# ducha-aiki/mods

Measured on AMD Instinct MI355X. Metric: image-pairs/sec (1024x768, HessAff+RootSIFT over the affine view ladder, MFMA FGINN match, LO-RANSAC H), higher is better.
Workload: dtype f32 (detect/describe) + u8 on the int8 matrix cores (distance matrix)

## Files before the change

mods_amd/csrc/engine.hip:

```cpp
#include <atomic>
#include <math.h>
#include <stdio.h>
#include <algorithm>
#include <chrono>
#include <map>
#include <unordered_set>
#include <mutex>
#include <dlfcn.h>
#include <string>
#include "engine_api.hpp"

#ifdef MODSX_DUP_BUILD
namespace mx {
int dup_count(int cls) {
  static const long mask = getenv("MODSX_DUP") ? strtol(getenv("MODSX_DUP"), nullptr, 0) : 0;
  return 1 + (int)((mask >> cls) & 1);
}
}
#endif
namespace mx {

static thread_local std::string g_err;
void set_error(const std::string &s) { g_err = s; }
static std::atomic<int> g_busyContexts{0};
// ... 362 lines not shown

static int cv_round(double v) { return (int)lrint(v); }

struct SigmaPlan {
  int levels;
  float sigmaStep;
  float curSigma[8];
  float incSigma[8];
};

static SigmaPlan make_sigma_plan(const modsx_hessaff_params &p) {
  SigmaPlan s;
  s.levels = p.numberOfScales + 2;
  s.sigmaStep = powf(2.0f, 1.0f / (float)p.numberOfScales);
  float cur = p.initialSigma;
  s.curSigma[0] = cur; s.incSigma[0] = 0;
  for (int i = 1; i < s.levels; i++) {
    s.incSigma[i] = cur * sqrtf(s.sigmaStep * s.sigmaStep - 1.0f);
    cur *= s.sigmaStep;
    s.curSigma[i] = cur;
  }
  return s;
}

static int fill_taps(BlurBatch &b, float sigma) {
  int n = blur_ksize(sigma);
  if (n > MAX_TAPS) { set_error("pyramid blur kernel larger than 17 taps is not supported"); return MODSX_ERR_ARG; }
  std::vector<float> k = gaussian_kernel(n, sigma);
  b.n = n;
  for (int i = 0; i < n; i++) b.k[i] = k[i];
  return MODSX_OK;
}

int build_pyramids(modsx_ctx *c, const modsx_image *const *imgs, int n, const modsx_hessaff_params &p,
                   bool singleOctaveFromFirstLevel) {
  if (n <= 0 || n > MAXB) { set_error("batch size"); return MODSX_ERR_ARG; }
  if (p.numberOfScales < 1 || p.numberOfScales > 6) { set_error("numberOfScales"); return MODSX_ERR_ARG; }
  if (p.detectorType != MODSX_DET_HESSIAN && p.detectorType != MODSX_DET_DOG && p.detectorType != MODSX_DET_HARRIS) {
    set_error("detectorType must be Hessian (0), DoG (1) or Harris (2)");
    return MODSX_ERR_ARG;
  }
  const bool hess = p.detectorType == MODSX_DET_HESSIAN;
  const SigmaPlan sp = make_sigma_plan(p);
  const int L = sp.levels;
  const int minSize = 2 * p.border + 2;
  int maxOct = 0;
  for (int i = 0; i < n; i++) {
    Pyramid &py = c->pyr[i];
    py.nOct = 0;
    int rows = imgs[i]->rows, cols = imgs[i]->cols;
    float pd = 1.0f;
    size_t total = 0;
    while (rows > minSize && cols > minSize && py.nOct < 24) {
      Octave &o = py.oct[py.nOct++];
      o.rows = rows; o.cols = cols; o.pixelDistance = pd;
      total += (size_t)2 * L * rows * cols;
      pd *= 2.0;
      rows = cv_round(rows * 0.5); cols = cv_round(cols * 0.5);
      if (singleOctaveFromFirstLevel) break;
    }
    if (!py.store.ensure(total * sizeof(float) + 64)) return MODSX_ERR_NOMEM;
    float *ptr = (float *)py.store.p;
    for (int o = 0; o < py.nOct; o++) {
      size_t npx = (size_t)py.oct[o].rows * py.oct[o].cols;
      for (int l = 0; l < L; l++) { py.oct[o].blur[l] = ptr; ptr += npx; }
      for (int l = 0; l < L; l++) { py.oct[o].resp[l] = ptr; ptr += npx; }
    }
    maxOct = std::max(maxOct, py.nOct);
  }
  hipStream_t s = c->stream;
  for (int o = 0; o < maxOct; o++) {
    BlurBatch bb;
    memset(&bb, 0, sizeof bb);
    int nj = 0, mr = 0, mc = 0;
    if (o == 0) {
      const float curSigma0 = 0.5f;
      const bool preBlur = !singleOctaveFromFirstLevel && p.initialSigma > curSigma0;
      if (preBlur) {
        float sigma = sqrtf(p.initialSigma * p.initialSigma - curSigma0 * curSigma0);
        int rc = fill_taps(bb, sigma);
        if (rc) return rc;
      }
      for (int i = 0; i < n; i++) {
        if (c->pyr[i].nOct <= 0) continue;
        Octave &oc = c->pyr[i].oct[0];
        BlurJob &j = bb.j[nj++];
        j.src = imgs[i]->d; j.blur = oc.blur[0]; j.resp = hess ? oc.resp[0] : nullptr; j.rows = oc.rows; j.cols = oc.cols;
        j.norm = sp.curSigma[0] * sp.curSigma[0];
        mr = std::max(mr, oc.rows); mc = std::max(mc, oc.cols);
        if (!preBlur) {
          MX_HIP(hipMemcpyAsync(oc.blur[0], imgs[i]->d, (size_t)oc.rows * oc.cols * 4, hipMemcpyDeviceToDevice, s));
          j.src = oc.blur[0];
        }
      }
      double px = 0;
      for (int q = 0; q < nj; q++) px += (double)bb.j[q].rows * bb.j[q].cols;
      if (nj) {
        if (preBlur) { ProfScope ps(c, K_BLUR_HESS, px * 12); launch_blur_hess(s, bb, nj, mr, mc); }
        else if (hess) { ProfScope ps(c, K_HESSIAN, px * 8); launch_hessian(s, bb, nj, mr, mc); }
      }
    } else {
      ResizeBatch rb;
      memset(&rb, 0, sizeof rb);
      for (int i = 0; i < n; i++) {
        if (c->pyr[i].nOct <= o) continue;
        Octave &pv = c->pyr[i].oct[o - 1], &oc = c->pyr[i].oct[o];
        ResizeJob &r = rb.j[nj];
        r.src = pv.blur[p.numberOfScales]; r.dst = oc.blur[0];
        r.srows = pv.rows; r.scols = pv.cols; r.drows = oc.rows; r.dcols = oc.cols;
        r.resp = hess ? oc.resp[0] : nullptr; r.norm = sp.curSigma[0] * sp.curSigma[0];
        BlurJob &j = bb.j[nj++];
        j.src = oc.blur[0]; j.blur = nullptr; j.resp = oc.resp[0]; j.rows = oc.rows; j.cols = oc.cols;
        j.norm = sp.curSigma[0] * sp.curSigma[0];
        mr = std::max(mr, oc.rows); mc = std::max(mc, oc.cols);
      }
      if (nj) {
        double spx = 0, dpx = 0;
        for (int q = 0; q < nj; q++) { spx += (double)rb.j[q].srows * rb.j[q].scols; dpx += (double)rb.j[q].drows * rb.j[q].dcols; }
        { ProfScope ps(c, K_RESIZE, (spx + dpx) * 4 + dpx * 4); launch_resize_half(s, rb, nj, mr, mc); }
      }
    }
    if (!nj) continue;
    for (int l = 1; l < L; l++) {
      BlurBatch b2;
      memset(&b2, 0, sizeof b2);
      int rc = fill_taps(b2, sp.incSigma[l]);
      if (rc) return rc;
      int k = 0;
      for (int i = 0; i < n; i++) {
        if (c->pyr[i].nOct <= o) continue;
        Octave &oc = c->pyr[i].oct[o];
        BlurJob &j = b2.j[k++];
        j.src = oc.blur[l - 1]; j.blur = oc.blur[l]; j.resp = hess ? oc.resp[l] : nullptr; j.rows = oc.rows; j.cols = oc.cols;
        j.norm = sp.curSigma[l] * sp.curSigma[l];
      }
      double px = 0;
      for (int q = 0; q < k; q++) px += (double)b2.j[q].rows * b2.j[q].cols;
      ProfScope ps(c, K_BLUR_HESS, px * 12);
      launch_blur_hess(s, b2, k, mr, mc);
    }
    if (!hess) {
      for (int l = 0; l < L; l++) {
        const float norm = sp.curSigma[l] * sp.curSigma[l];
        const float sigma = p.detectorType == MODSX_DET_DOG ? norm : sqrtf((float)(0.6 * norm));
        const int nt = blur_ksize(sigma);
        if (2 * nt > 2 * 4096) { set_error("response blur kernel too large"); return MODSX_ERR_ARG; }
        if (!c->viewTaps.ensure((size_t)L * 2 * 4100 * 4) || !c->hViewTaps.ensure((size_t)L * 2 * 4100 * 4)) return MODSX_ERR_NOMEM;
        float *dT = (float *)c->viewTaps.p + (size_t)l * 2 * 4100, *hT = (float *)c->hViewTaps.p + (size_t)l * 2 * 4100;
        bool tapsUp = false;
        for (int i = 0; i < n; i++) {
          if (c->pyr[i].nOct <= o) continue;
          Octave &oc = c->pyr[i].oct[o];
          const int rows = oc.rows, cols = oc.cols;
          const size_t npx = (size_t)rows * cols;
          if (!c->scratchA.ensure(npx * 4 * 8)) return MODSX_ERR_NOMEM;
          float *buf = (float *)c->scratchA.p, *tmp = buf, *a = buf + npx, *b = buf + 2 * npx, *cc = buf + 3 * npx;
          float *ba = buf + 4 * npx, *bb2 = buf + 5 * npx, *bc = buf + 6 * npx;
          const int nx = cols == 1 ? 1 : nt, ny = rows == 1 ? 1 : nt;
          if (!tapsUp || nx != nt || ny != nt) {
            std::vector<float> kx = gaussian_kernel(nx, sigma), ky = gaussian_kernel(ny, sigma);
            if (tapsUp) MX_HIP(ctx_sync(c));
            memcpy(hT, kx.data(), nx * 4); memcpy(hT + nx, ky.data(), ny * 4);
            MX_HIP(ctx_copy(c, dT, hT, (size_t)(nx + ny) * 4, hipMemcpyHostToDevice));
            tapsUp = nx == nt && ny == nt;
          }
          auto blur = [&](const float *src, float *dst) {
            if (nt == 1) { MX_HIP(hipMemcpyAsync(dst, src, npx * 4, hipMemcpyDeviceToDevice, s)); return MODSX_OK; }
            launch_blur_pass(s, src, tmp, rows, cols, dT, nx, 0, 1);
            launch_blur_pass(s, tmp, dst, rows, cols, dT + nx, ny, 1, 1);
            return MODSX_OK;
          };
          if (p.detectorType == MODSX_DET_DOG) {
            int rc = blur(oc.blur[l], a);
            if (rc) return rc;
            launch_sub(s, oc.blur[l], a, oc.resp[l], npx);
          } else {
            launch_grad_products(s, oc.blur[l], rows, cols, a, b, cc);
            int rc = blur(a, ba);
            if (!rc) rc = blur(b, bb2);
            if (!rc) rc = blur(cc, bc);
            if (rc) return rc;
            launch_harris_combine(s, ba, bb2, bc, (float)(0.6 * norm), oc.resp[l], npx);
          }
        }
      }
    }
  }
  MX_HIP(hipGetLastError());
  return MODSX_OK;
}

static const unsigned CAND_CAP = 1u << 21;

int detect_scalespace_batch(modsx_ctx *c, const modsx_image *const *imgs, int n, const modsx_hessaff_params &p,
                            std::vector<modsx_sskp> *out) {
  int rc = build_pyramids(c, imgs, n, p, false);
  if (rc) return rc;
  hipStream_t s = c->stream;
  if (!c->cand.ensure((size_t)CAND_CAP * sizeof(Candidate)) || !c->nmsQueue.ensure((size_t)CAND_CAP * 16)) return MODSX_ERR_NOMEM;
  if (!c->counter.ensure((NMS_QUEUES + 1) * 128)) return MODSX_ERR_NOMEM;
  MX_HIP(hipMemsetAsync(c->counter.p, 0, 128 + NMS_QUEUES * 128, s));
  bool queuesClean = true;
  NmsBatch nb;
  memset(&nb, 0, sizeof nb);
  nb.edgeScoreThreshold = (p.edgeEigenValueRatio + 1.0f) * (p.edgeEigenValueRatio + 1.0f) / p.edgeEigenValueRatio;
  float finalTh = p.threshold;
  float posTh = (float)(0.8 * finalTh);
  float negTh = -posTh;
  if (p.detectorType == MODSX_DET_HESSIAN) finalTh = p.threshold * p.threshold;
  if (p.mode != MODSX_FIXED_TH) finalTh = posTh = negTh = 0.0f;
  nb.posTh = posTh; nb.negTh = negTh; nb.finalTh = finalTh; nb.border = p.border; nb.detType = p.detectorType;
  int maxOct = 0;
  for (int i = 0; i < n; i++) maxOct = std::max(maxOct, c->pyr[i].nOct);
  const bool perOctave = p.numberOfScales == 3 && !getenv("MODSX_NMS_PER_LEVEL");
  std::vector<NmsJob> hjobs;
  std::vector<int> hpfx(1, 0), hfirst;
  double px = 0;
  auto flush = [&](bool last) -> int {
    const int nj = (int)hjobs.size();
    if (!nj) return MODSX_OK;
    const int np = (int)hpfx.size() - 1;
    const size_t jobBytes = (size_t)nj * sizeof(NmsJob), pfxBytes = (size_t)(np + 1) * 4, firstBytes = (size_t)std::max<size_t>(1, hfirst.size()) * 4;
    if (!c->nmsJobs.ensure(jobBytes + pfxBytes + firstBytes + 64)) return MODSX_ERR_NOMEM;
    if (!c->hNms.ensure(jobBytes + pfxBytes + firstBytes)) return MODSX_ERR_NOMEM;
    memcpy(c->hNms.p, hjobs.data(), jobBytes);
    memcpy((char *)c->hNms.p + jobBytes, hpfx.data(), pfxBytes);
    if (!hfirst.empty()) memcpy((char *)c->hNms.p + jobBytes + pfxBytes, hfirst.data(), hfirst.size() * 4);
    MX_HIP(ctx_copy(c, c->nmsJobs.p, c->hNms.p, jobBytes + pfxBytes + firstBytes, hipMemcpyHostToDevice));
    if (!c->tileJob.ensure((size_t)hpfx.back() * 4 + 4)) return MODSX_ERR_NOMEM;
    const int *dPfx = (const int *)((char *)c->nmsJobs.p + jobBytes);
    launch_expand_tiles(s, dPfx, np, (int *)c->tileJob.p);
    {
      ProfScope ps(c, K_NMS, px * 12);
      if (!queuesClean) MX_HIP(hipMemsetAsync((unsigned *)c->counter.p + 32, 0, NMS_QUEUES * 128, s));
      queuesClean = false;
      launch_nms(s, nb, (const NmsJob *)c->nmsJobs.p, dPfx, (const int *)c->tileJob.p, nj,
                 hpfx.back(), (int4 *)c->nmsQueue.p, (unsigned *)c->counter.p + 32, CAND_CAP, (Candidate *)c->cand.p,
                 (unsigned *)c->counter.p, CAND_CAP, perOctave ? (const int *)((char *)c->nmsJobs.p + jobBytes + pfxBytes) : nullptr,
                 p.numberOfScales);
    }
    if (!last) MX_HIP(ctx_sync(c));
    hjobs.clear(); hpfx.assign(1, 0); hfirst.clear(); px = 0;
    return MODSX_OK;
  };
  for (int o = 0; o < maxOct; o++)
    for (int i = 0; i < n; i++) {
      if (c->pyr[i].nOct <= o) continue;
      Octave &oc = c->pyr[i].oct[o];
      const int w = oc.cols - 2 * p.border, h = oc.rows - 2 * p.border;
      if (w <= 0 || h <= 0) continue;
      if ((int)hjobs.size() + p.numberOfScales > NMS_MAXJ) { int rcf = flush(false); if (rcf) return rcf; }
      const int tiles = ((w + 63) / 64) * ((h + NMS_TILE_ROWS - 1) / NMS_TILE_ROWS);
      if (perOctave) { hfirst.push_back((int)hjobs.size()); hpfx.push_back(hpfx.back() + tiles); }
      for (int l = 1; l <= p.numberOfScales; l++) {
        NmsJob j;
        j.low = oc.resp[l - 1]; j.cur = oc.resp[l]; j.high = oc.resp[l + 1]; j.blur = oc.blur[l];
        j.rows = oc.rows; j.cols = oc.cols; j.img = i; j.octave = o; j.level = l; j.pad = 0;
        hjobs.push_back(j);
        if (!perOctave) hpfx.push_back(hpfx.back() + tiles);
        px += (double)oc.rows * oc.cols;
      }
    }
  { int rcf = flush(true); if (rcf) return rcf; }
  static const bool deviceOrder = getenv("MODSX_DEVICE_ORDER") != nullptr && atoi(getenv("MODSX_DEVICE_ORDER")) != 0;
  if (deviceOrder) {
    typedef size_t (*temp_fn)(unsigned);
    typedef int (*order_fn)(hipStream_t, const Candidate *, const unsigned *, unsigned, unsigned long long *, unsigned long long *, unsigned *, unsigned *,
                            void *, size_t, unsigned long long *, unsigned *, unsigned, unsigned *, Candidate *, unsigned *);
    static temp_fn cand_sort_temp_bytes = nullptr;
    static order_fn launch_cand_order = nullptr;
    static std::once_flag candOnce;
    std::call_once(candOnce, [] {
      Dl_info di;
      std::string path = "libmodsx_cand.so";
      if (dladdr((const void *)&modsx_create, &di) && di.dli_fname) {
        const std::string self(di.dli_fname);
        const size_t sl = self.rfind('/');
        if (sl != std::string::npos) path = self.substr(0, sl + 1) + "libmodsx_cand.so";
// ... 1195 lines not shown
```

mods_amd/csrc/engine.hpp:

```cpp
#pragma once
#include <hip/hip_runtime.h>
#include <stdint.h>
#include <stdlib.h>
#include <string.h>
#include <string>
#include <vector>
#include "../../include/modsx.h"
#include "kmath.hpp"

namespace mx {

#ifndef MODSX_MAXB
#define MODSX_MAXB 32
#endif
constexpr int MAXB = MODSX_MAXB;
constexpr int PAIR_GROUP = 4;
constexpr int NMS_MAXJ = 1024;
constexpr int MAX_TAPS = 17;

struct BlurJob {
  const float *src;
  float *blur;
  float *resp;
  int rows, cols;
  float norm;
  int pad;
};
struct BlurBatch {
  int n;
  float k[MAX_TAPS];
  BlurJob j[MAXB];
  int nj;
  int tile0[MAXB + 1];
};
struct ResizeJob {
  const float *src;
  float *dst;
  float *resp;
  int srows, scols, drows, dcols;
  float norm;
  int pad;
};
struct ResizeBatch { ResizeJob j[MAXB]; int nj; int tile0[MAXB + 1]; };
struct NmsJob {
  const float *low, *cur, *high, *blur;
  int rows, cols, img, octave, level, pad;
};
struct NmsBatch {
  float posTh, negTh, finalTh;
  int border;
  double edgeScoreThreshold;
  int detType, pad;
};
struct Candidate {
  int img, octave, level, type;
  int r0, c0, r, c;
  float b0, b1, b2, val;
};

struct AffJob {
  const float *blur;
  int rows, cols;
  float x, y, s, pixelDistance;
};
struct AffOut { float u11, u12, u21, u22; int ok; int iters; };

struct OriJob {
// ... 51 lines not shown
};

struct MatchRow {
  int t0, t1, nless, nbad;
  int tj;
  float dj;
  float d0, d1;
};
static_assert(sizeof(MatchRow) == 32, "match rows are 32 bytes");

struct DevBuf {
  void *p = nullptr;
  size_t cap = 0;
  bool ensure(size_t bytes);
  void release();
};
struct PinBuf {
  void *p = nullptr;
  size_t cap = 0;
  bool ensure(size_t bytes);
  void release();
};

struct Octave {
  int rows, cols;
  float pixelDistance;
  float *blur[8];
  float *resp[8];
};
struct Pyramid {
  int nOct = 0;
  Octave oct[24];
  DevBuf store;
};

void set_error(const std::string &s);
bool gpu_shared();
struct CtxBusy { modsx_ctx *c; explicit CtxBusy(modsx_ctx *c); ~CtxBusy(); CtxBusy(const CtxBusy &) = delete; CtxBusy &operator=(const CtxBusy &) = delete; };
hipError_t ctx_copy(modsx_ctx *c, void *dst, const void *src, size_t bytes, hipMemcpyKind kind);
hipError_t ctx_sync(modsx_ctx *c);
unsigned ctx_mark(modsx_ctx *c);
bool ctx_mark_reached(modsx_ctx *c, unsigned seq);
hipError_t ctx_wait_mark(modsx_ctx *c, unsigned seq);
bool host_wait_runtime();
int host_cpus_per_rank();
#define MX_HIP(expr)                                                                          \
  do {                                                                                        \
    hipError_t e_ = (expr);                                                                   \
    if (e_ != hipSuccess) {                                                                   \
      mx::set_error(std::string(#expr) + ": " + hipGetErrorString(e_));                       \
      return MODSX_ERR_DEVICE;                                                                \
    }                                                                                         \
  } while (0)

std::vector<float> gaussian_kernel(int n, double sigma);
int blur_ksize(float sigma);
void gauss_mask(float *mask, int size);
void circular_gauss_mask(float *mask, int size, float sigma);
const double *atan_lut_host();
inline bool check_borders_host(int w, int h, float ofsx, float ofsy, float a11, float a12, float a21, float a22, int rw, int rh) {
  return check_borders(w, h, ofsx, ofsy, a11, a12, a21, a22, rw, rh);
}
bool invert3(const double *S, double *t);
void rectify(double &a11, double &a12, double &a21, double &a22);

void launch_blur_hess(hipStream_t s, const BlurBatch &b, int nj, int maxRows, int maxCols);
void launch_hessian(hipStream_t s, const BlurBatch &b, int nj, int maxRows, int maxCols);
void launch_resize_half(hipStream_t s, const ResizeBatch &b, int nj, int maxRows, int maxCols);
void launch_nms(hipStream_t s, const NmsBatch &b, const NmsJob *jobs, const int *tilePrefix, const int *tileJob, int nj,
                int nTiles, int4 *queue, unsigned *qcount, unsigned qcap, Candidate *out, unsigned *counter, unsigned cap,
                const int *octFirst = nullptr, int levelsPerOctave = 0);
size_t cand_sort_temp_bytes(unsigned nsort);
int launch_cand_order(hipStream_t s, const Candidate *cand, const unsigned *counter, unsigned nsort, unsigned long long *keys,
                      unsigned long long *keys2, unsigned *idx, unsigned *idx2, void *temp, size_t tempBytes, unsigned long long *tabKey,
                      unsigned *tabRank, unsigned tabSize, unsigned *slotOf, Candidate *out, unsigned *outCount);
constexpr int NMS_QUEUES = 64;
constexpr int NMS_TILE_ROWS = 16;
void launch_gray(hipStream_t s, const void *src, float *dst, size_t n, int channels, int dtype);
void launch_baumberg(hipStream_t s, const AffJob *jobs, AffOut *out, int n, const float *mask, int W, int maxIter,
                     float convTh, float affInitialSigma);
constexpr int ATAN_CASES = 2048 + 64;
constexpr int ORI_NV = 1344;
void launch_orientation(hipStream_t s, const OriJob *jobs, float *out, int n, const ImgRef *imgs,
                        const unsigned short *maskIdx, const float *maskW,
                        const unsigned char *binTab, int doHalf, double th, int maxAngles);
void launch_trunc_u8(hipStream_t s, const float *src, uint8_t *dst, size_t n);
size_t mser_sort_blocks(const int *rows, int n);
void launch_mser_sort(hipStream_t s, const uint8_t *const *u8, const int *rows, const int *cols, const size_t *ordOfs, int n, int *blockHist,
                      int *start, int *order);
void launch_expand_blur_tiles(hipStream_t s, const DescJob *jobs, const int *prefixRows, const int *prefixCols, int nJobs,
                              const int *needTab, BlurTile *tilesRows, BlurTile *tilesCols, float2 *rowStarts);
void launch_sample_rows(hipStream_t s, const DescJob *jobs, const BlurTile *tiles, int nTiles, const ImgRef *imgs, const float *taps,
                        const int *needTab, float *dst, const float2 *rowStarts, float *dstGrid);
void launch_blur_cols(hipStream_t s, const BlurTile *tiles, int nTiles, const float *taps, const int *needTab, const float *src,
                      float *dst);
void launch_expand_tiles(hipStream_t s, const int *prefix, int nJobs, int *tileJob);
void launch_patch_sample(hipStream_t s, const DescJob *jobs, const int *tilePrefix, const int *tileJob, int nTiles,
                         const ImgRef *imgs, float *scratch);
void launch_patch_blur(hipStream_t s, const DescJob *jobs, const int *tilePrefix, const int *tileJob, int nTiles,
                       const float *taps, const int *needTab, const float *src, float *dst, int pass);
void launch_describe(hipStream_t s, const DescJob *jobs, int n, const ImgRef *imgs, const float *grid,
                     const int *needTab, const float *coordTab,
                     const float *mask, const unsigned short *maskIdx, int nmask, const float *oTab, const int *bins,
                     const double *wts, int photoNorm, int descTypes, int nOut, double maxBin, const DescOut &outs);
// ... 121 lines not shown
```

mods_amd/csrc/engine_api.hpp:

```cpp
#pragma once
#include <functional>
#include <string>
#include <vector>
#include "engine.hpp"

struct modsx_comm;

namespace mx {
const char *last_error();
void prof_collect(modsx_ctx *c);
void prof_reset(modsx_ctx *c, bool enable);
modsx_ctx *ctx_create(int device_id);
void ctx_destroy(modsx_ctx *c);
int build_pyramids(modsx_ctx *c, const modsx_image *const *imgs, int n, const modsx_hessaff_params &p,
                   bool singleOctaveFromFirstLevel);
int detect_scalespace_batch(modsx_ctx *c, const modsx_image *const *imgs, int n, const modsx_hessaff_params &p,
                            std::vector<modsx_sskp> *out);
int detect_keypoints_batch(modsx_ctx *c, const modsx_image *const *imgs, int n, const modsx_hessaff_params &par,
                           const double *tilts, const double *zooms, std::vector<modsx_keypoint> *out);
void detect_affine_regions(const modsx_keypoint *kps, int n, int img_id, int det_type, modsx_region *out);
int detect_orientation_batch(modsx_ctx *c, const modsx_image *const *imgs, int n, const std::vector<modsx_region> *in,
                             double mrSize, int patchSize, int doHalfSIFT, int maxAngNum, double th, int addUpRight,
                             std::vector<modsx_region> *out);
int reproject_regions(modsx_region *regs, int n, const double *H, int orig_w, int orig_h);
int reproject_regions_box(modsx_region *regs, int n, const double *H, int orig_w, int orig_h, double boxk);
struct DescSet {
  int n = 1;
  int type[MODSX_MAX_DESC] = {MODSX_DESC_ROOT_SIFT, 0, 0, 0};
  double ratio[MODSX_MAX_DESC] = {0, 0, 0, 0};
  bool forceHalf = false;
  bool half() const { for (int i = 0; i < n; i++) if (type[i] >= 2) return true; return forceHalf; }
  int packed() const { int p = 0; for (int i = 0; i < n; i++) p |= (type[i] & 15) << (4 * i); return p; }
};
int resolve_descs(const modsx_pair_params &pp, const modsx_ladder_step *st, DescSet &ds);
void desc_class_order(const DescSet &ds, int *ord);
int describe_batch(modsx_ctx *c, const modsx_image *const *imgs, int n, const std::vector<modsx_region> *regs,
                   double mrSize, int patchSize, int fast, int photoNorm, int descType, double maxBin,
                   float *const *descHost, float *const *devF, uint8_t *const *devU8, const DescSet *ds = nullptr,
                   uint8_t *const *const *devU8x = nullptr);
struct ProfScopeFwd;
int set_vs_pars(const double *scale_set, int ns, const double *tilt_set, int nt, double phi_base, double InitSigma,
                int doBlur, modsx_view *par, int cap, modsx_view *prev, int *nprev, int cap_prev);
int synth_view(modsx_ctx *c, const modsx_image *gray, const modsx_view &v, modsx_image **out, double *H, int *identity,
               int slot = -1);
int detect_describe_items(modsx_ctx *c, const modsx_image *const *itemImg, const int *itemView, int nitems, const modsx_view *views,
                          const modsx_pair_params &pp, std::vector<modsx_region> &regs,
                          float *devF, uint8_t *devU8, size_t devCapRegions, float *hostDesc, int *itemCounts,
                          const DescSet *ds = nullptr, uint8_t *const *devU8x = nullptr);
// ... 115 lines not shown
```

mods_amd/csrc/kernels_pyramid.hip:

```cpp
#include "engine.hpp"

namespace mx {

constexpr int TW = 64;
constexpr int TMP_W = TW + 4;

MX_D int find_job(const int *tile0, int nj, int t) {
  int j = 0;
  while (j + 1 < nj && t >= tile0[j + 1]) j++;
  return j;
}

typedef float f2 __attribute__((ext_vector_type(2)));

template <int R, int TH>
__global__ __launch_bounds__(256) void k_blur_hess(BlurBatch batch) {
  constexpr int BLR_H = TH + 4;
  const int ji = find_job(batch.tile0, batch.nj, blockIdx.x);
  const BlurJob jb = batch.j[ji];
  const int rows = jb.rows, cols = jb.cols;
  const int lt = blockIdx.x - batch.tile0[ji], ntx = (cols + TW - 1) / TW;
  const int tx0 = (lt % ntx) * TW, ty0 = (lt / ntx) * TH;
  constexpr int n = 2 * R + 1;
  constexpr int sh = BLR_H + 2 * R, sw = TMP_W + 2 * R;
  static_assert(sh % 2 == 0, "the input tile is parked as row pairs");
  constexpr int SW = (sw + 3) & ~3;
  __shared__ __attribute__((aligned(16))) float src[sh * SW];
  __shared__ __attribute__((aligned(16))) float tmp[sh * TMP_W];
  float *blr = src;
  const int tid = threadIdx.x;
  {
    constexpr int PER = (sh * sw + 255) / 256;
    float t[PER];
#pragma unroll
    for (int u = 0; u < PER; u++) {
      const int i = tid + 256 * u, ii = i < sh * sw ? i : sh * sw - 1;
      const int ly = ii / sw, lx = ii - ly * sw;
      int gy = ty0 - 1 - R + ly, gx = tx0 - 1 - R + lx;
      gy = gy < 0 ? 0 : (gy > rows - 1 ? rows - 1 : gy);
      gx = gx < 0 ? 0 : (gx > cols - 1 ? cols - 1 : gx);
      t[u] = as_global(jb.src)[__umul24((unsigned)gy, (unsigned)cols) + (unsigned)gx];
    }
#pragma unroll
    for (int u = 0; u < PER; u++) {
      const int i = tid + 256 * u;
      if (i < sh * sw) { const int ly = i / sw, lx = i - ly * sw; src[(ly >> 1) * (2 * SW) + 2 * lx + (ly & 1)] = t[u]; }
    }
  }
  __syncthreads();
  for (int i = tid; i < (sh / 2) * (TMP_W / 4); i += 256) {
    const int lp = i / (TMP_W / 4), g = i - lp * (TMP_W / 4);
    const f2 *S = reinterpret_cast<const f2 *>(src) + lp * SW + 4 * g;
    f2 w[4 + 2 * R];
#pragma unroll
    for (int q = 0; q < (4 + 2 * R) / 2; q++) {
      const float4 t = *reinterpret_cast<const float4 *>(S + 2 * q);
      w[2 * q] = (f2){t.x, t.y}; w[2 * q + 1] = (f2){t.z, t.w};
    }
    f2 v[4];
#pragma unroll
    for (int o = 0; o < 4; o++) {
      if (n <= 5) {
        v[o] = w[o + R] * batch.k[R];
#pragma unroll
        for (int j = 1; j <= R; j++) v[o] = v[o] + (w[o + R - j] + w[o + R + j]) * batch.k[R + j];
      } else {
        v[o] = (f2){0.f, 0.f};
#pragma unroll
        for (int j = 0; j < n; j++) v[o] = v[o] + w[o + j] * batch.k[j];
      }
    }
    *reinterpret_cast<float4 *>(tmp + (2 * lp) * TMP_W + 4 * g) = make_float4(v[0].x, v[1].x, v[2].x, v[3].x);
    *reinterpret_cast<float4 *>(tmp + (2 * lp + 1) * TMP_W + 4 * g) = make_float4(v[0].y, v[1].y, v[2].y, v[3].y);
  }
  __syncthreads();
  for (int i = tid; i < (BLR_H / 4) * (TMP_W / 2); i += 256) {
    const int gy = i / (TMP_W / 2), lx = 2 * (i - gy * (TMP_W / 2));
    const float *S = tmp + (4 * gy) * TMP_W + lx;
    f2 w[4 + 2 * R];
#pragma unroll
    for (int q = 0; q < 4 + 2 * R; q++) w[q] = *reinterpret_cast<const f2 *>(S + q * TMP_W);
#pragma unroll
    for (int o = 0; o < 4; o++) {
      f2 v = w[o + R] * batch.k[R] + (f2){0.f, 0.f};
#pragma unroll
      for (int j = 1; j <= R; j++) v = v + (w[o + R + j] + w[o + R - j]) * batch.k[R + j];
      *reinterpret_cast<f2 *>(blr + (4 * gy + o) * TMP_W + lx) = v;
    }
  }
  __syncthreads();
  const float norm2 = jb.norm * jb.norm;
  for (int i = tid; i < TH * TW; i += 256) {
    const int ly = i / TW, lx = i - ly * TW;
    const int gy = ty0 + ly, gx = tx0 + lx;
    if (gy >= rows || gx >= cols) continue;
    const float *B = blr + (ly + 1) * TMP_W + (lx + 1);
    const unsigned gofs = __umul24((unsigned)gy, (unsigned)cols) + (unsigned)gx;
    jb.blur[gofs] = B[0];
    if (jb.resp) {
      float o = 0.f;
      if (gy >= 1 && gy < rows - 1 && gx >= 1 && gx < cols - 1) {
        const float v11 = B[-TMP_W - 1], v12 = B[-TMP_W], v13 = B[-TMP_W + 1];
        const float v21 = B[-1], v22 = B[0], v23 = B[1];
        const float v31 = B[TMP_W - 1], v32 = B[TMP_W], v33 = B[TMP_W + 1];
        float Lxx = (v21 - 2 * v22 + v23);
        float Lyy = (v12 - 2 * v22 + v32);
        float Lxy = (v13 - v11 + v31 - v33) / 4.0f;
        o = (Lxx * Lyy - Lxy * Lxy) * norm2;
      }
      jb.resp[gofs] = o;
    }
  }
}

__global__ __launch_bounds__(256) void k_hessian(BlurBatch batch) {
  const int ji = find_job(batch.tile0, batch.nj, blockIdx.x);
  const BlurJob jb = batch.j[ji];
  const int rows = jb.rows, cols = jb.cols;
  const int lt = blockIdx.x - batch.tile0[ji], ntx = (cols + 63) / 64;
  const int gx = (lt % ntx) * 64 + (threadIdx.x & 63), gy = (lt / ntx) * 4 + (threadIdx.x >> 6);
  if (gx >= cols || gy >= rows) return;
  float o = 0.f;
  if (gy >= 1 && gy < rows - 1 && gx >= 1 && gx < cols - 1) {
    const float *B = jb.src + (size_t)gy * cols + gx;
    const float v11 = B[-cols - 1], v12 = B[-cols], v13 = B[-cols + 1];
    const float v21 = B[-1], v22 = B[0], v23 = B[1];
    const float v31 = B[cols - 1], v32 = B[cols], v33 = B[cols + 1];
    float Lxx = (v21 - 2 * v22 + v23);
    float Lyy = (v12 - 2 * v22 + v32);
    float Lxy = (v13 - v11 + v31 - v33) / 4.0f;
    o = (Lxx * Lyy - Lxy * Lxy) * (jb.norm * jb.norm);
  }
  jb.resp[(size_t)gy * cols + gx] = o;
}

MX_D float resize_half_px(const float *src, int sr, int sc, int dx, int dy) {
  const int sy0 = dy * 2, sx0 = dx * 2;
  float out;
  if (sy0 >= sr) out = 0.f;
  else if (sy0 + 2 <= sr && dx < sc / 2) {
    const float *S = src + (size_t)sy0 * sc + sx0;
    float sum = 0.f;
    sum = sum + (((S[0] + S[1]) + S[sc]) + S[sc + 1]);
// ... 368 lines not shown
  unsigned n = qcount[32 * sq];
  n = n < qsub ? n : qsub;
  const int lane = threadIdx.x & 63;
  for (unsigned i0 = blockIdx.x * 256; i0 < n; i0 += gridDim.x * 256) {
    const unsigned i = i0 + threadIdx.x;
    Candidate k;
    bool ok = false;
    if (i < n) {
      const int4 q = queue[(size_t)sq * qsub + i];
      ok = nms_refine(batch, jobs[q.x], q.y, q.z, k);
    }
    const unsigned long long m = __ballot(ok);
    if (m) {
      unsigned base = 0;
      const int leader = __ffsll((long long)m) - 1;
      if (lane == leader) base = atomicAdd(counter, (unsigned)__popcll(m));
      base = __shfl(base, leader);
      const unsigned slot = base + (unsigned)__popcll(m & ((1ull << lane) - 1ull));
      if (ok && slot < cap) out[slot] = k;
    }
  }
}

void launch_nms(hipStream_t s, const NmsBatch &b, const NmsJob *jobs, const int *tilePrefix, const int *tileJob, int nj,
                int nTiles, int4 *queue, unsigned *qcount, unsigned qcap, Candidate *out, unsigned *counter, unsigned cap,
                const int *octFirst, int levelsPerOctave) {
  if (nj <= 0 || nTiles <= 0) return;
  if (octFirst && levelsPerOctave == 3)
    hipLaunchKernelGGL(k_nms_localize_oct<3>, dim3(nTiles), dim3(256), 0, s, b, jobs, octFirst, tilePrefix, tileJob, queue, qcount, qcap, counter + 1);
  else
  hipLaunchKernelGGL(k_nms_localize, dim3(nTiles), dim3(256), 0, s, b, jobs, tilePrefix, tileJob, queue, qcount, qcap, counter + 1);
  hipLaunchKernelGGL(k_nms_refine, dim3(NMS_REFINE_BLOCKS, NMS_QUEUES), dim3(256), 0, s, b, jobs, queue, qcount, qcap, out, counter, cap);
}
__global__ void k_trunc_u8(const float *src, uint8_t *dst, size_t n) {
  const size_t i = ((size_t)blockIdx.x * blockDim.x + threadIdx.x) * 4;
  if (i + 3 < n) {
    const float4 v = *reinterpret_cast<const float4 *>(src + i);
    const unsigned p = (unsigned)(uint8_t)v.x | ((unsigned)(uint8_t)v.y << 8) | ((unsigned)(uint8_t)v.z << 16) | ((unsigned)(uint8_t)v.w << 24);
    *reinterpret_cast<unsigned *>(dst + i) = p;
  } else {
    for (size_t k = i; k < n; k++) dst[k] = (uint8_t)src[k];
  }
}
void launch_trunc_u8(hipStream_t s, const float *src, uint8_t *dst, size_t n) {
  if (!n) return;
  const size_t threads = (n + 3) / 4;
  hipLaunchKernelGGL(k_trunc_u8, dim3((unsigned)((threads + 255) / 256)), dim3(256), 0, s, src, dst, n);
}
constexpr int MSB_ROWS = 8;
struct MserSortBatch {
  const uint8_t *u8[MAXB];
  int rows[MAXB], cols[MAXB], blk0[MAXB + 1];
  unsigned long long ordOfs[MAXB];
  int n;
};
MX_D int mser_view_of(const MserSortBatch &b, int blk) {
  int v = 0;
  while (v + 1 < b.n && blk >= b.blk0[v + 1]) v++;
  return v;
}
__global__ __launch_bounds__(64) void k_mser_hist(MserSortBatch b, int *blockHist) {
  __shared__ int h[256];
  const int blk = blockIdx.x, v = mser_view_of(b, blk), lane = threadIdx.x;
  for (int i = lane; i < 256; i += 64) h[i] = 0;
  __syncthreads();
  const int r0 = (blk - b.blk0[v]) * MSB_ROWS, r1 = min(r0 + MSB_ROWS, b.rows[v]), cols = b.cols[v];
// ... 74 lines not shown
```

Before: 217.7.

## Fuse NMS scan and next-octave seeding into the blur-Hessian pyramid kernel

The blur+Hessian kernel now does more of the detector's work itself. It runs the scale-space extremum scan on the previous level while the current response tile is still in shared memory, and pushes candidates straight into the NMS refine queues. It also writes the next octave's half-resolution base level and its Hessian response from the last blurred level, which removes the separate resize pass. The global tile load is restructured into per-wave row loads. This removes the separate localize kernel and the extra passes over response and blur memory, at the cost of a heavier, more register- and shared-memory-hungry kernel, more complex code, and an environment variable to fall back to the old path.

Result: slower. 208.8 (-4.1%).

```diff
diff --git a/mods_amd/csrc/engine.hip b/mods_amd/csrc/engine.hip
--- a/mods_amd/csrc/engine.hip
+++ b/mods_amd/csrc/engine.hip
@@ -418,19 +418,27 @@
   return MODSX_OK;
 }
 
-int build_pyramids(modsx_ctx *c, const modsx_image *const *imgs, int n, const modsx_hessaff_params &p,
-                   bool singleOctaveFromFirstLevel) {
+enum { PYR_SEP_SCAN = 1, PYR_SEP_SEED = 2 };
+static int pyramid_separate() {
+#ifdef MODSX_DUP_BUILD
+  return PYR_SEP_SCAN | PYR_SEP_SEED;
+#endif
+  const char *e = getenv("MODSX_PYRAMID_SEPARATE");
+  if (!e || !*e || !strcmp(e, "0")) return 0;
+  if (!strcmp(e, "scan")) return PYR_SEP_SCAN;
+  if (!strcmp(e, "seed")) return PYR_SEP_SEED;
+  return PYR_SEP_SCAN | PYR_SEP_SEED;
+}
+
+int plan_pyramids(modsx_ctx *c, const modsx_image *const *imgs, int n, const modsx_hessaff_params &p, bool singleOctaveFromFirstLevel) {
   if (n <= 0 || n > MAXB) { set_error("batch size"); return MODSX_ERR_ARG; }
   if (p.numberOfScales < 1 || p.numberOfScales > 6) { set_error("numberOfScales"); return MODSX_ERR_ARG; }
   if (p.detectorType != MODSX_DET_HESSIAN && p.detectorType != MODSX_DET_DOG && p.detectorType != MODSX_DET_HARRIS) {
     set_error("detectorType must be Hessian (0), DoG (1) or Harris (2)");
     return MODSX_ERR_ARG;
   }
-  const bool hess = p.detectorType == MODSX_DET_HESSIAN;
-  const SigmaPlan sp = make_sigma_plan(p);
-  const int L = sp.levels;
+  const int L = p.numberOfScales + 2;
   const int minSize = 2 * p.border + 2;
-  int maxOct = 0;
   for (int i = 0; i < n; i++) {
     Pyramid &py = c->pyr[i];
     py.nOct = 0;
@@ -452,8 +460,19 @@
       for (int l = 0; l < L; l++) { py.oct[o].blur[l] = ptr; ptr += npx; }
       for (int l = 0; l < L; l++) { py.oct[o].resp[l] = ptr; ptr += npx; }
     }
-    maxOct = std::max(maxOct, py.nOct);
-  }
+  }
+  return MODSX_OK;
+}
+
+int build_pyramids(modsx_ctx *c, const modsx_image *const *imgs, int n, const modsx_hessaff_params &p,
+                   bool singleOctaveFromFirstLevel, const PyramidScan *scan) {
+  if (!scan) { int rc = plan_pyramids(c, imgs, n, p, singleOctaveFromFirstLevel); if (rc) return rc; }
+  const bool hess = p.detectorType == MODSX_DET_HESSIAN;
+  const bool seed = hess && p.numberOfScales == 3 && !singleOctaveFromFirstLevel && !(pyramid_separate() & PYR_SEP_SEED);
+  const SigmaPlan sp = make_sigma_plan(p);
+  const int L = sp.levels;
+  int maxOct = 0;
+  for (int i = 0; i < n; i++) maxOct = std::max(maxOct, c->pyr[i].nOct);
   hipStream_t s = c->stream;
   for (int o = 0; o < maxOct; o++) {
     BlurBatch bb;
@@ -500,7 +519,7 @@
         j.norm = sp.curSigma[0] * sp.curSigma[0];
         mr = std::max(mr, oc.rows); mc = std::max(mc, oc.cols);
       }
-      if (nj) {
+      if (nj && !seed) {
         double spx = 0, dpx = 0;
         for (int q = 0; q < nj; q++) { spx += (double)rb.j[q].srows * rb.j[q].scols; dpx += (double)rb.j[q].drows * rb.j[q].dcols; }
         { ProfScope ps(c, K_RESIZE, (spx + dpx) * 4 + dpx * 4); launch_resize_half(s, rb, nj, mr, mc); }
@@ -519,6 +538,18 @@
         BlurJob &j = b2.j[k++];
         j.src = oc.blur[l - 1]; j.blur = oc.blur[l]; j.resp = hess ? oc.resp[l] : nullptr; j.rows = oc.rows; j.cols = oc.cols;
         j.norm = sp.curSigma[l] * sp.curSigma[l];
+        if (seed && l == p.numberOfScales && c->pyr[i].nOct > o + 1) {
+          Octave &nx = c->pyr[i].oct[o + 1];
+          j.nextBlur = nx.blur[0]; j.nextResp = nx.resp[0]; j.nrows = nx.rows; j.ncols = nx.cols;
+          j.nextNorm = sp.curSigma[0] * sp.curSigma[0];
+        }
+        if (scan && hess && l >= 2 && scan->jobOf[i][o] >= 0) {
+          j.scanLow = oc.resp[l - 2]; j.scanCur = oc.resp[l - 1]; j.scanJob = scan->jobOf[i][o] + l - 2;
+        }
+      }
+      if (scan) {
+        b2.posTh = scan->posTh; b2.negTh = scan->negTh; b2.border = scan->border; b2.qcap = scan->qcap;
+        b2.queue = scan->queue; b2.qcount = scan->qcount; b2.overflow = scan->overflow;
       }
       double px = 0;
       for (int q = 0; q < k; q++) px += (double)b2.j[q].rows * b2.j[q].cols;
@@ -580,7 +611,7 @@
 
 int detect_scalespace_batch(modsx_ctx *c, const modsx_image *const *imgs, int n, const modsx_hessaff_params &p,
                             std::vector<modsx_sskp> *out) {
-  int rc = build_pyramids(c, imgs, n, p, false);
+  int rc = plan_pyramids(c, imgs, n, p, false);
   if (rc) return rc;
   hipStream_t s = c->stream;
   if (!c->cand.ensure((size_t)CAND_CAP * sizeof(Candidate)) || !c->nmsQueue.ensure((size_t)CAND_CAP * 16)) return MODSX_ERR_NOMEM;
@@ -602,6 +633,48 @@
   std::vector<NmsJob> hjobs;
   std::vector<int> hpfx(1, 0), hfirst;
   double px = 0;
+  bool fusedScan = perOctave && p.detectorType == MODSX_DET_HESSIAN && p.border >= 1 && !(pyramid_separate() & PYR_SEP_SCAN);
+  if (fusedScan) {
+    int total = 0;
+    for (int i = 0; i < n; i++) total += c->pyr[i].nOct * p.numberOfScales;
+    fusedScan = total > 0 && total <= NMS_MAXJ;
+  }
+  if (fusedScan) {
+    PyramidScan ps;
+    memset(&ps, 0, sizeof ps);
+    ps.posTh = posTh; ps.negTh = negTh; ps.border = p.border; ps.qcap = CAND_CAP;
+    ps.queue = (int4 *)c->nmsQueue.p; ps.qcount = (unsigned *)c->counter.p + 32; ps.overflow = (unsigned *)c->counter.p + 1;
+    for (int o = 0; o < maxOct; o++)
+      for (int i = 0; i < n; i++) {
+        if (c->pyr[i].nOct <= o) continue;
+        Octave &oc = c->pyr[i].oct[o];
+        ps.jobOf[i][o] = -1;
+        if (oc.cols - 2 * p.border <= 0 || oc.rows - 2 * p.border <= 0) continue;
+        ps.jobOf[i][o] = (int)hjobs.size();
+        for (int l = 1; l <= p.numberOfScales; l++) {
+          NmsJob j;
+          j.low = oc.resp[l - 1]; j.cur = oc.resp[l]; j.high = oc.resp[l + 1]; j.blur = oc.blur[l];
+          j.rows = oc.rows; j.cols = oc.cols; j.img = i; j.octave = o; j.level = l; j.pad = 0;
+          hjobs.push_back(j);
+          px += (double)oc.rows * oc.cols;
+        }
+      }
+    const size_t jobBytes = hjobs.size() * sizeof(NmsJob);
+    if (!c->nmsJobs.ensure(jobBytes + 64) || !c->hNms.ensure(jobBytes + 64)) return MODSX_ERR_NOMEM;
+    memcpy(c->hNms.p, hjobs.data(), jobBytes);
+    if (jobBytes) MX_HIP(ctx_copy(c, c->nmsJobs.p, c->hNms.p, jobBytes, hipMemcpyHostToDevice));
+    rc = build_pyramids(c, imgs, n, p, false, &ps);
+    if (rc) return rc;
+    if (!hjobs.empty()) {
+      ProfScope pr(c, K_NMS, px * 12);
+      launch_nms_refine(s, nb, (const NmsJob *)c->nmsJobs.p, (const int4 *)c->nmsQueue.p, (const unsigned *)c->counter.p + 32, CAND_CAP,
+                        (Candidate *)c->cand.p, (unsigned *)c->counter.p, CAND_CAP);
+    }
+    hjobs.clear(); px = 0;
+  } else {
+    rc = build_pyramids(c, imgs, n, p, false);
+    if (rc) return rc;
+  }
   auto flush = [&](bool last) -> int {
     const int nj = (int)hjobs.size();
     if (!nj) return MODSX_OK;
@@ -629,7 +702,7 @@
     hjobs.clear(); hpfx.assign(1, 0); hfirst.clear(); px = 0;
     return MODSX_OK;
   };
-  for (int o = 0; o < maxOct; o++)
+  for (int o = 0; o < maxOct && !fusedScan; o++)
     for (int i = 0; i < n; i++) {
       if (c->pyr[i].nOct <= o) continue;
       Octave &oc = c->pyr[i].oct[o];
diff --git a/mods_amd/csrc/engine.hpp b/mods_amd/csrc/engine.hpp
--- a/mods_amd/csrc/engine.hpp
+++ b/mods_amd/csrc/engine.hpp
@@ -24,6 +24,11 @@
   float *resp;
   int rows, cols;
   float norm;
+  int scanJob;
+  const float *scanLow, *scanCur;
+  float *nextBlur, *nextResp;
+  int nrows, ncols;
+  float nextNorm;
   int pad;
 };
 struct BlurBatch {
@@ -32,7 +37,13 @@
   BlurJob j[MAXB];
   int nj;
   int tile0[MAXB + 1];
-};
+  float posTh, negTh;
+  int border;
+  unsigned qcap;
+  int4 *queue;
+  unsigned *qcount, *overflow;
+};
+static_assert(sizeof(BlurBatch) <= 3584, "kernel arguments: 4 KB at most");
 struct ResizeJob {
   const float *src;
   float *dst;
@@ -150,6 +161,15 @@
   int nOct = 0;
   Octave oct[24];
   DevBuf store;
+};
+
+struct PyramidScan {
+  int jobOf[MAXB][24];
+  float posTh, negTh;
+  int border;
+  unsigned qcap;
+  int4 *queue;
+  unsigned *qcount, *overflow;
 };
 
 void set_error(const std::string &s);
@@ -188,6 +208,8 @@
 void launch_nms(hipStream_t s, const NmsBatch &b, const NmsJob *jobs, const int *tilePrefix, const int *tileJob, int nj,
                 int nTiles, int4 *queue, unsigned *qcount, unsigned qcap, Candidate *out, unsigned *counter, unsigned cap,
                 const int *octFirst = nullptr, int levelsPerOctave = 0);
+void launch_nms_refine(hipStream_t s, const NmsBatch &b, const NmsJob *jobs, const int4 *queue, const unsigned *qcount, unsigned qcap,
+                       Candidate *out, unsigned *counter, unsigned cap);
 size_t cand_sort_temp_bytes(unsigned nsort);
 int launch_cand_order(hipStream_t s, const Candidate *cand, const unsigned *counter, unsigned nsort, unsigned long long *keys,
                       unsigned long long *keys2, unsigned *idx, unsigned *idx2, void *temp, size_t tempBytes, unsigned long long *tabKey,
diff --git a/mods_amd/csrc/engine_api.hpp b/mods_amd/csrc/engine_api.hpp
--- a/mods_amd/csrc/engine_api.hpp
+++ b/mods_amd/csrc/engine_api.hpp
@@ -12,8 +12,10 @@
 void prof_reset(modsx_ctx *c, bool enable);
 modsx_ctx *ctx_create(int device_id);
 void ctx_destroy(modsx_ctx *c);
+struct PyramidScan;
+int plan_pyramids(modsx_ctx *c, const modsx_image *const *imgs, int n, const modsx_hessaff_params &p, bool singleOctaveFromFirstLevel);
 int build_pyramids(modsx_ctx *c, const modsx_image *const *imgs, int n, const modsx_hessaff_params &p,
-                   bool singleOctaveFromFirstLevel);
+                   bool singleOctaveFromFirstLevel, const PyramidScan *scan = nullptr);
 int detect_scalespace_batch(modsx_ctx *c, const modsx_image *const *imgs, int n, const modsx_hessaff_params &p,
                             std::vector<modsx_sskp> *out);
 int detect_keypoints_batch(modsx_ctx *c, const modsx_image *const *imgs, int n, const modsx_hessaff_params &par,
diff --git a/mods_amd/csrc/kernels_pyramid.hip b/mods_amd/csrc/kernels_pyramid.hip
--- a/mods_amd/csrc/kernels_pyramid.hip
+++ b/mods_amd/csrc/kernels_pyramid.hip
@@ -12,6 +12,29 @@
 }
 
 typedef float f2 __attribute__((ext_vector_type(2)));
+
+MX_D int clampi(int v, int hi) { return min(max(v, 0), hi); }
+MX_D float hess9(float v11, float v12, float v13, float v21, float v22, float v23, float v31, float v32, float v33, float norm2) {
+  float Lxx = (v21 - 2 * v22 + v23);
+  float Lyy = (v12 - 2 * v22 + v32);
+  float Lxy = (v13 - v11 + v31 - v33) / 4.0f;
+  return (Lxx * Lyy - Lxy * Lxy) * norm2;
+}
+MX_D float resize_half_blk(float s00, float s01, float s10, float s11, int sr, int sc, int sy0, int sx0) {
+  if (sy0 + 2 <= sr && (sx0 >> 1) < sc / 2) {
+    float sum = 0.f;
+    sum = sum + (((s00 + s01) + s10) + s11);
+    return sum * 0.25f;
+  }
+  float sum = 0.f; int count = 0;
+  sum += s00; count++;
+  if (sx0 + 1 < sc) { sum += s01; count++; }
+  if (sy0 + 1 < sr) {
+    sum += s10; count++;
+    if (sx0 + 1 < sc) { sum += s11; count++; }
+  }
+  return sum / (float)count;
+}
 
 template <int R, int TH>
 __global__ __launch_bounds__(256) void k_blur_hess(BlurBatch batch) {
@@ -28,23 +51,33 @@
   __shared__ __attribute__((aligned(16))) float src[sh * SW];
   __shared__ __attribute__((aligned(16))) float tmp[sh * TMP_W];
   float *blr = src;
-  const int tid = threadIdx.x;
+  const int tid = threadIdx.x, lane = tid & 63;
+  const int wv = __builtin_amdgcn_readfirstlane(tid >> 6);
   {
-    constexpr int PER = (sh * sw + 255) / 256;
-    float t[PER];
-#pragma unroll
-    for (int u = 0; u < PER; u++) {
-      const int i = tid + 256 * u, ii = i < sh * sw ? i : sh * sw - 1;
-      const int ly = ii / sw, lx = ii - ly * sw;
-      int gy = ty0 - 1 - R + ly, gx = tx0 - 1 - R + lx;
-      gy = gy < 0 ? 0 : (gy > rows - 1 ? rows - 1 : gy);
-      gx = gx < 0 ? 0 : (gx > cols - 1 ? cols - 1 : gx);
-      t[u] = as_global(jb.src)[__umul24((unsigned)gy, (unsigned)cols) + (unsigned)gx];
-    }
-#pragma unroll
-    for (int u = 0; u < PER; u++) {
-      const int i = tid + 256 * u;
-      if (i < sh * sw) { const int ly = i / sw, lx = i - ly * sw; src[(ly >> 1) * (2 * SW) + 2 * lx + (ly & 1)] = t[u]; }
+    constexpr int NR = (sh + 3) / 4, TAIL = sw - 64;
+    static_assert(TAIL > 0 && TAIL <= 64, "two columns per lane");
+    float t0[NR], t1[NR];
+    typedef const char __attribute__((address_space(1))) *gbyte_p;
+    const unsigned bx0 = 4u * (unsigned)clampi(tx0 - 2 - R + lane, cols - 1), bx1 = 4u * (unsigned)clampi(tx0 - 2 - R + 64 + lane, cols - 1);
+    const bool tail = lane < TAIL;
+    auto row_ptr = [&](int u) {
+      const int ly = (4 * u + 3 < sh) ? wv + 4 * u : min(wv + 4 * u, sh - 1);
+      return (gbyte_p)(as_global(jb.src) + (unsigned)clampi(ty0 - 2 - R + ly, rows - 1) * (unsigned)cols);
+    };
+#pragma unroll
+    for (int u = 0; u < NR; u++) { t0[u] = *(gcfloat_p)(row_ptr(u) + bx0); t1[u] = 0.f; }
+    if (tail) {
+#pragma unroll
+      for (int u = 0; u < NR; u++) t1[u] = *(gcfloat_p)(row_ptr(u) + bx1);
+    }
+    float *d = src + (wv >> 1) * (2 * SW) + (wv & 1) + 2 * lane;
+#pragma unroll
+    for (int u = 0; u < NR; u++)
+      if (4 * u + 3 < sh || wv + 4 * u < sh) d[u * 4 * SW] = t0[u];
+    if (tail) {
+#pragma unroll
+      for (int u = 0; u < NR; u++)
+        if (4 * u + 3 < sh || wv + 4 * u < sh) d[u * 4 * SW + 128] = t1[u];
     }
   }
   __syncthreads();
@@ -89,26 +122,129 @@
     }
   }
   __syncthreads();
-  const float norm2 = jb.norm * jb.norm;
-  for (int i = tid; i < TH * TW; i += 256) {
-    const int ly = i / TW, lx = i - ly * TW;
-    const int gy = ty0 + ly, gx = tx0 + lx;
+  float *rsp = tmp;
+  unsigned *qc = reinterpret_cast<unsigned *>(tmp + (TH + 2) * TMP_W);
+  static_assert((TH + 2) * TMP_W + 2 <= sh * TMP_W, "response ring + queue words fit the row-filtered tile");
+  if (jb.resp) {
+    const float norm2 = jb.norm * jb.norm;
+    for (int i = tid; i < ((TH + 2) / 2) * (TW + 2); i += 256) {
+      const int g = i / (TW + 2), rx = i - g * (TW + 2), ry = 2 * g;
+      const float *B = blr + ry * TMP_W + rx;
+      float a[4][3];
+#pragma unroll
+      for (int q = 0; q < 4; q++)
+#pragma unroll
+        for (int e = 0; e < 3; e++) a[q][e] = B[q * TMP_W + e];
+      const int gx = tx0 - 1 + rx;
+#pragma unroll
+      for (int o = 0; o < 2; o++) {
+        const int gy = ty0 - 1 + ry + o;
+        float v = 0.f;
+        if (gy >= 1 && gy < rows - 1 && gx >= 1 && gx < cols - 1)
+          v = hess9(a[o][0], a[o][1], a[o][2], a[o + 1][0], a[o + 1][1], a[o + 1][2], a[o + 2][0], a[o + 2][1], a[o + 2][2], norm2);
+        rsp[(ry + o) * TMP_W + rx] = v;
+      }
+    }
+    if (tid == 0) qc[0] = 0;
+    __syncthreads();
+  }
+  const int gx = tx0 + lane;
+#pragma unroll
+  for (int u = 0; u < TH / 4; u++) {
+    const int ly = (tid >> 6) + 4 * u, gy = ty0 + ly;
     if (gy >= rows || gx >= cols) continue;
-    const float *B = blr + (ly + 1) * TMP_W + (lx + 1);
     const unsigned gofs = __umul24((unsigned)gy, (unsigned)cols) + (unsigned)gx;
-    jb.blur[gofs] = B[0];
-    if (jb.resp) {
+    jb.blur[gofs] = blr[(ly + 2) * TMP_W + lane + 2];
+    if (jb.resp) jb.resp[gofs] = rsp[(ly + 1) * TMP_W + lane + 1];
+  }
+  if (jb.scanCur && jb.resp) {
+    const int B = batch.border;
+    const float posTh = batch.posTh, negTh = batch.negTh;
+    float v0[TH / 4];
+    unsigned pass = 0;
+#pragma unroll
+    for (int u = 0; u < TH / 4; u++) {
+      const int gy = ty0 + (tid >> 6) + 4 * u;
+      v0[u] = 0.f;
+      if (gy >= B && gy < rows - B && gx >= B && gx < cols - B) {
+        v0[u] = as_global(jb.scanCur)[__umul24((unsigned)gy, (unsigned)cols) + (unsigned)gx];
+        pass |= 1u << u;
+      }
+    }
+    unsigned hit = 0, found = 0;
+#pragma unroll
+    for (int u = 0; u < TH / 4; u++)
+      if (((pass >> u) & 1u) && (v0[u] > posTh || v0[u] < negTh)) hit |= 1u << u;
+    while (hit) {
+      const int u = __ffs(hit) - 1;
+      hit &= hit - 1;
+      const int ly = (tid >> 6) + 4 * u;
+      const unsigned gofs = __umul24((unsigned)(ty0 + ly), (unsigned)cols) + (unsigned)gx;
+      const float v = as_global(jb.scanCur)[gofs];
+      float mx = v, mn = v;
+#pragma unroll
+      for (int dr = -1; dr <= 1; dr++)
+#pragma unroll
+        for (int dc = -1; dc <= 1; dc++) {
+          const unsigned o = gofs + (unsigned)(dr * cols + dc);
+          const float a = as_global(jb.scanLow)[o], b = as_global(jb.scanCur)[o], h = rsp[(ly + 1 + dr) * TMP_W + lane + 1 + dc];
+          mx = fmaxf(mx, fmaxf(fmaxf(a, b), h));
+          mn = fminf(mn, fminf(fminf(a, b), h));
+        }
+      bool cand = false;
+      if (v > posTh) cand = mx <= v;
+      else if (v < negTh) cand = mn >= v;
+      if (cand) found |= 1u << u;
+    }
+    const unsigned cnt = __popc(found);
+    unsigned slot = 0;
+    if (cnt) slot = atomicAdd(&qc[0], cnt);
+    __syncthreads();
+    const unsigned sq = blockIdx.x % NMS_QUEUES, qsub = batch.qcap / NMS_QUEUES;
+    if (tid == 0) qc[1] = qc[0] ? atomicAdd(batch.qcount + 32 * sq, qc[0]) : 0u;
+    __syncthreads();
+    if (cnt) {
+      slot += qc[1];
+#pragma unroll
+      for (int u = 0; u < TH / 4; u++)
+        if ((found >> u) & 1u) {
+          if (slot < qsub) batch.queue[(size_t)sq * qsub + slot] = make_int4(jb.scanJob, ty0 + (tid >> 6) + 4 * u, gx, 0);
+          else atomicOr(batch.overflow, 1u);
+          slot++;
+        }
+    }
+  }
+  if (jb.nextBlur) {
+    constexpr int HH = TH / 2 + 2, HW = TW / 2 + 2, HS = HW + 2;
+    static_assert(HH * HS <= sh * TMP_W, "half-resolution tile fits the row-filtered tile");
+    float *hf = tmp;
+    __syncthreads();
+    for (int i = tid; i < HH * HW; i += 256) {
+      const int hy = i / HW, hx = i - hy * HW;
+      const int sy0 = ty0 - 2 + 2 * hy, sx0 = tx0 - 2 + 2 * hx;
       float o = 0.f;
-      if (gy >= 1 && gy < rows - 1 && gx >= 1 && gx < cols - 1) {
-        const float v11 = B[-TMP_W - 1], v12 = B[-TMP_W], v13 = B[-TMP_W + 1];
-        const float v21 = B[-1], v22 = B[0], v23 = B[1];
-        const float v31 = B[TMP_W - 1], v32 = B[TMP_W], v33 = B[TMP_W + 1];
-        float Lxx = (v21 - 2 * v22 + v23);
-        float Lyy = (v12 - 2 * v22 + v32);
-        float Lxy = (v13 - v11 + v31 - v33) / 4.0f;
-        o = (Lxx * Lyy - Lxy * Lxy) * norm2;
-      }
-      jb.resp[gofs] = o;
+      if (sy0 >= 0 && sx0 >= 0 && sy0 < rows && sx0 < cols) {
+        const float *P = blr + (2 * hy) * TMP_W + 2 * hx;
+        o = resize_half_blk(P[0], P[1], P[TMP_W], P[TMP_W + 1], rows, cols, sy0, sx0);
+      }
+      hf[hy * HS + hx] = o;
+    }
+    __syncthreads();
+    const int drows = jb.nrows, dcols = jb.ncols;
+    const float nnorm2 = jb.nextNorm * jb.nextNorm;
+    for (int i = tid; i < (TH / 2) * (TW / 2); i += 256) {
+      const int hy = i / (TW / 2), hx = i - hy * (TW / 2);
+      const int dy = ty0 / 2 + hy, dx = tx0 / 2 + hx;
+      if (dy >= drows || dx >= dcols) continue;
+      const float *H = hf + (hy + 1) * HS + hx + 1;
+      const unsigned dofs = __umul24((unsigned)dy, (unsigned)dcols) + (unsigned)dx;
+      jb.nextBlur[dofs] = H[0];
+      if (jb.nextResp) {
+        float o = 0.f;
+        if (dy >= 1 && dy < drows - 1 && dx >= 1 && dx < dcols - 1)
+          o = hess9(H[-HS - 1], H[-HS], H[-HS + 1], H[-1], H[0], H[1], H[HS - 1], H[HS], H[HS + 1], nnorm2);
+        jb.nextResp[dofs] = o;
+      }
     }
   }
 }
@@ -543,6 +679,10 @@
   hipLaunchKernelGGL(k_nms_localize, dim3(nTiles), dim3(256), 0, s, b, jobs, tilePrefix, tileJob, queue, qcount, qcap, counter + 1);
   hipLaunchKernelGGL(k_nms_refine, dim3(NMS_REFINE_BLOCKS, NMS_QUEUES), dim3(256), 0, s, b, jobs, queue, qcount, qcap, out, counter, cap);
 }
+void launch_nms_refine(hipStream_t s, const NmsBatch &b, const NmsJob *jobs, const int4 *queue, const unsigned *qcount, unsigned qcap,
+                       Candidate *out, unsigned *counter, unsigned cap) {
+  hipLaunchKernelGGL(k_nms_refine, dim3(NMS_REFINE_BLOCKS, NMS_QUEUES), dim3(256), 0, s, b, jobs, queue, qcount, qcap, out, counter, cap);
+}
 __global__ void k_trunc_u8(const float *src, uint8_t *dst, size_t n) {
   const size_t i = ((size_t)blockIdx.x * blockDim.x + threadIdx.x) * 4;
   if (i + 3 < n) {
```
